# PathologyFoundation/plip

Measured on NVIDIA H100. Metric: image-text pairs/sec (224x224, 77-tok), higher is better.
Workload: dtype bf16

## Files before the change

### plip_b200/csrc/gemm_wgmma.cu

```cuda
#include "gemm.cuh"
#include "wgmma.cuh"

#include <stdio.h>
#include <stdlib.h>

namespace plip {

namespace {

constexpr int BM = 64;
constexpr int BK = 64;
constexpr int kThreads = 288;
constexpr int kConsumerWarps = 8;
constexpr uint32_t A_STAGE = BM * BK * 2;
constexpr uint32_t kStoreStageBytes = 16 * 128;

constexpr int x_boxes(int BN, int EPI) {
  return EPI != EPI_BIAS_RESID_F32 ? 2 : BN == 192 ? 3 : 2;
}

template <int BN, int EPI>
struct Cfg {
  static constexpr uint32_t B_STAGE = BN * BK * 2;
  static constexpr uint32_t STAGE = A_STAGE + B_STAGE;
  static constexpr int XBOXES = x_boxes(BN, EPI);
  static constexpr uint32_t EPI_BYTES = kConsumerWarps * XBOXES * kStoreStageBytes;
  static constexpr uint32_t BAR_BYTES = EPI == EPI_BIAS_RESID_F32 ? 512 : 256;
  static constexpr uint32_t ALIGN_SLACK = 1024;
  static constexpr int kMaxStages = (227 * 1024 - BAR_BYTES - EPI_BYTES - ALIGN_SLACK) / STAGE;
  static constexpr int STAGES = kMaxStages > 8 ? 8 : kMaxStages;
  static constexpr uint32_t SMEM_BYTES = STAGES * STAGE + EPI_BYTES + BAR_BYTES + ALIGN_SLACK;
};

struct GemmDev {
  int M, N, K;
  const float* bias;
  const float* rowscale;
  void* out;
  int ldo;
  const float* pos;
  int patches, seq;
  const float* colsum;
  const float2* stats_in;
  int n_partials;
  __nv_bfloat16* xb_out;
  float2* stats_out;
};

template <bool F16, int BN>
__device__ __forceinline__ void wgmma_ss(float (&d)[BN / 2], uint64_t adesc, uint64_t bdesc, uint32_t scale_d) {
  if constexpr (BN == 128) wgmma_ss_n128<F16>(d, adesc, bdesc, scale_d);
  else if constexpr (BN == 192) wgmma_ss_n192<F16>(d, adesc, bdesc, scale_d);
  else wgmma_ss_n256<F16>(d, adesc, bdesc, scale_d);
}

__device__ __forceinline__ float2 ln_row_terms(const GemmDev& p, int grow) {
  float s1 = 0.f, s2 = 0.f;
#pragma unroll
  for (int j = 0; j < kStatSlots; ++j) {
    const float2 t = (grow < p.M && j < p.n_partials) ? __ldg(p.stats_in + static_cast<size_t>(grow) * kStatSlots + j)
                                                      : make_float2(0.f, 0.f);
    s1 += t.x;
    s2 += t.y;
  }
  const float inv_k = 1.0f / static_cast<float>(p.K);
  const float mean = s1 * inv_k;
  const float rstd = rsqrtf(fmaxf(s2 * inv_k - mean * mean, 0.f) + kLnEps);
  return make_float2(-rstd * mean, rstd);
}

template <int BN, int EPI, bool F16>
__device__ __forceinline__ void epilogue_warp(const GemmDev& p, const CUtensorMap* tmC, float (&d)[BN / 2], uint32_t stage_smem,
                                              uint32_t& stage_sel, uint32_t xbar, int row_base, int col_base, int n_blk, int lane,
                                              float2 ln0, float2 ln1) {
  constexpr bool LN_FOLD = (EPI == EPI_LN_BIAS_BF16 || EPI == EPI_LN_BIAS_GELU_BF16);
  constexpr bool GELU = (EPI == EPI_BIAS_GELU_BF16 || EPI == EPI_LN_BIAS_GELU_BF16);
  constexpr bool HAS_BIAS = (EPI == EPI_BIAS_BF16 || EPI == EPI_BIAS_GELU_BF16 || EPI == EPI_BIAS_RESID_F32 || LN_FOLD);
  constexpr bool OUT_BF16 = (EPI == EPI_BIAS_BF16 || EPI == EPI_BIAS_GELU_BF16 || LN_FOLD);
  const int q = lane & 3, rr = lane >> 2;
  const int row0 = row_base + rr, row1 = row0 + 8;

  if constexpr (EPI == EPI_NULL) {
    float acc = 0.f;
#pragma unroll
    for (int i = 0; i < BN / 2; ++i) acc += d[i];
    if (acc == 1.2345e30f && p.M < 0) reinterpret_cast<float*>(p.out)[0] = acc;
  } else if constexpr (OUT_BF16) {
#pragma unroll
    for (int blk = 0; blk < BN / 64; ++blk) {
      const uint32_t buf = stage_smem + (stage_sel & 1u) * kStoreStageBytes;
      ++stage_sel;
      if (lane == 0) tma_store_wait_read_but_one();
      __syncwarp();
#pragma unroll
      for (int jj = 0; jj < 8; ++jj) {
        const int j = blk * 8 + jj;
        const int col = col_base + 8 * j + 2 * q;
        const float2 b = __ldg(reinterpret_cast<const float2*>(p.bias + col));
        float v00 = d[4 * j + 0], v01 = d[4 * j + 1], v10 = d[4 * j + 2], v11 = d[4 * j + 3];
        if constexpr (LN_FOLD) {
          const float2 cs = __ldg(reinterpret_cast<const float2*>(p.colsum + col));
          v00 = fmaf(ln0.y, v00, fmaf(ln0.x, cs.x, b.x));
          v01 = fmaf(ln0.y, v01, fmaf(ln0.x, cs.y, b.y));
          v10 = fmaf(ln1.y, v10, fmaf(ln1.x, cs.x, b.x));
          v11 = fmaf(ln1.y, v11, fmaf(ln1.x, cs.y, b.y));
        } else {
          v00 += b.x; v01 += b.y; v10 += b.x; v11 += b.y;
        }
        if constexpr (GELU) {
          v00 = quick_gelu(v00); v01 = quick_gelu(v01); v10 = quick_gelu(v10); v11 = quick_gelu(v11);
        }
        st_shared_b32(buf + rr * 128 + ((jj ^ rr) << 4) + q * 4, pack_op2<F16>(v00, v01));
        st_shared_b32(buf + (rr + 8) * 128 + ((jj ^ rr) << 4) + q * 4, pack_op2<F16>(v10, v11));
      }
      fence_proxy_async_smem();
      __syncwarp();
      if (lane == 0) {
        tma_store_2d(tmC, buf, col_base + blk * 64, row_base);
        tma_store_commit();
      }
    }
  } else if constexpr (EPI == EPI_BIAS_RESID_F32) {
    constexpr int kChunkCols = 32;
    constexpr int kChunks = BN / kChunkCols;
    constexpr int NB = x_boxes(BN, EPI);
    static_assert(kChunks % NB == 0, "every tile must start at staging block 0");
    constexpr int kUses = kChunks / NB;
    const bool ok0 = row0 < p.M, ok1 = row1 < p.M;
    const bool emit = p.xb_out != nullptr;
    const size_t o0 = static_cast<size_t>(ok0 ? row0 : 0) * p.ldo + col_base + 2 * q;
    const size_t o1 = o0 + 8 * static_cast<size_t>(p.ldo);
    uint32_t ph0 = 0;
    if constexpr (kUses % 2 != 0) ph0 = stage_sel++ & 1u;
    auto fetch = [&](int c) {
      if (lane == 0) {
        const uint32_t bar = xbar + 8u * (c % NB);
        mbar_arrive_expect_tx(bar, kStoreStageBytes);
        tma_load_2d(stage_smem + (c % NB) * kStoreStageBytes, tmC, bar, 2 * (col_base + c * kChunkCols), row_base);
      }
    };
    if (lane == 0) tma_store_wait_read();
    __syncwarp();
#pragma unroll
    for (int c = 0; c < NB; ++c) fetch(c);
    float st[2][2] = {};
#pragma unroll
    for (int c = 0; c < kChunks; ++c) {
      const int h = c < kChunks / 2 ? 0 : 1;
      mbar_wait(xbar + 8u * (c % NB), ph0 ^ ((c / NB) & 1u));
      const uint32_t buf = stage_smem + (c % NB) * kStoreStageBytes;
#pragma unroll
      for (int jj = 0; jj < kChunkCols / 8; ++jj) {
        const int j = c * (kChunkCols / 8) + jj;
        const int col = col_base + 8 * j + 2 * q;
        const uint32_t xoff = (((2 * jj + (q >> 1)) ^ rr) << 4) + (q & 1) * 8;
        const float2 b = __ldg(reinterpret_cast<const float2*>(p.bias + col));
        const float2 v0 = make_float2(d[4 * j + 0] + b.x, d[4 * j + 1] + b.y);
        const float2 v1 = make_float2(d[4 * j + 2] + b.x, d[4 * j + 3] + b.y);
        if (ok0) {
          const float2 x = ld_shared_f32x2(buf + rr * 128 + xoff);
          const float2 y = make_float2(x.x + v0.x, x.y + v0.y);
          st_shared_f32x2(buf + rr * 128 + xoff, y);
          if (emit) {
            *reinterpret_cast<uint32_t*>(p.xb_out + o0 + 8 * j) = pack_op2<F16>(y.x, y.y);
            st[0][0] += y.x + y.y;
            st[0][1] = fmaf(y.x, y.x, fmaf(y.y, y.y, st[0][1]));
          }
        }
        if (ok1) {
          const float2 x = ld_shared_f32x2(buf + (rr + 8) * 128 + xoff);
          const float2 y = make_float2(x.x + v1.x, x.y + v1.y);
          st_shared_f32x2(buf + (rr + 8) * 128 + xoff, y);
          if (emit) {
            *reinterpret_cast<uint32_t*>(p.xb_out + o1 + 8 * j) = pack_op2<F16>(y.x, y.y);
            st[1][0] += y.x + y.y;
            st[1][1] = fmaf(y.x, y.x, fmaf(y.y, y.y, st[1][1]));
          }
        }
      }
      fence_proxy_async_smem();
      __syncwarp();
      if (lane == 0) {
        tma_store_2d(tmC, buf, 2 * (col_base + c * kChunkCols), row_base);
        tma_store_commit();
      }
      if (c + NB < kChunks) {
        if (lane == 0) tma_store_wait_read();
        fetch(c + NB);
      }
      if (emit && (c + 1) % (kChunks / 2) == 0) {
#pragma unroll
        for (int r = 0; r < 2; ++r) {
          float a = st[r][0], b = st[r][1];
#pragma unroll
          for (int o = 1; o < 4; o <<= 1) {
            a += __shfl_xor_sync(0xffffffffu, a, o);
            b += __shfl_xor_sync(0xffffffffu, b, o);
          }
          if (q == 0 && (r == 0 ? ok0 : ok1))
            p.stats_out[static_cast<size_t>(row0 + 8 * r) * kStatSlots + 2 * n_blk + h] = make_float2(a, b);
          st[r][0] = 0.f;
          st[r][1] = 0.f;
        }
      }
    }
  } else {
    float* out = reinterpret_cast<float*>(p.out);
    const bool ok0 = row0 < p.M, ok1 = row1 < p.M;
    float rs0 = 1.f, rs1 = 1.f;
    size_t o0 = static_cast<size_t>(ok0 ? row0 : 0) * p.ldo, o1 = static_cast<size_t>(ok1 ? row1 : 0) * p.ldo;
    if constexpr (EPI == EPI_SIM_F32) {
      rs0 = ok0 ? __ldg(p.rowscale + row0) : 0.f;
      rs1 = ok1 ? __ldg(p.rowscale + row1) : 0.f;
    }
    size_t q0 = 0, q1 = 0;
    if constexpr (EPI == EPI_PATCH_F32) {
      const int r0 = ok0 ? row0 : 0, r1 = ok1 ? row1 : 0;
      const int b0 = r0 / p.patches, b1 = r1 / p.patches;
      o0 = static_cast<size_t>(b0 * p.seq + 1 + (r0 - b0 * p.patches)) * p.ldo;
      o1 = static_cast<size_t>(b1 * p.seq + 1 + (r1 - b1 * p.patches)) * p.ldo;
      q0 = static_cast<size_t>(1 + (r0 - b0 * p.patches)) * p.N;
      q1 = static_cast<size_t>(1 + (r1 - b1 * p.patches)) * p.N;
    }
#pragma unroll
    for (int j = 0; j < BN / 8; ++j) {
      const int col = col_base + 8 * j + 2 * q;
      float2 v0 = make_float2(d[4 * j + 0], d[4 * j + 1]), v1 = make_float2(d[4 * j + 2], d[4 * j + 3]);
      if constexpr (HAS_BIAS) {
        const float2 b = __ldg(reinterpret_cast<const float2*>(p.bias + col));
        v0.x += b.x; v0.y += b.y; v1.x += b.x; v1.y += b.y;
      }
      if constexpr (EPI == EPI_SIM_F32) {
        const float2 cs = __ldg(reinterpret_cast<const float2*>(p.bias + col));
        if (ok0) *reinterpret_cast<float2*>(out + o0 + col) = make_float2(v0.x * rs0 * cs.x, v0.y * rs0 * cs.y);
        if (ok1) *reinterpret_cast<float2*>(out + o1 + col) = make_float2(v1.x * rs1 * cs.x, v1.y * rs1 * cs.y);
      } else if constexpr (EPI == EPI_PATCH_F32) {
        if (ok0) {
          const float2 e = __ldg(reinterpret_cast<const float2*>(p.pos + q0 + col));
          *reinterpret_cast<float2*>(out + o0 + col) = make_float2(v0.x + e.x, v0.y + e.y);
        }
        if (ok1) {
          const float2 e = __ldg(reinterpret_cast<const float2*>(p.pos + q1 + col));
          *reinterpret_cast<float2*>(out + o1 + col) = make_float2(v1.x + e.x, v1.y + e.y);
        }
      } else {
        if (ok0) *reinterpret_cast<float2*>(out + o0 + col) = v0;
        if (ok1) *reinterpret_cast<float2*>(out + o1 + col) = v1;
      }
    }
  }
}

template <int CG, int BN, int EPI, bool F16>
__global__ void __launch_bounds__(kThreads, 1)
gemm_kernel(const __grid_constant__ CUtensorMap tmA, const __grid_constant__ CUtensorMap tmB,
            const __grid_constant__ CUtensorMap tmC, const GemmDev p) {
  using C = Cfg<BN, EPI>;
  constexpr int STAGES = C::STAGES;
  extern __shared__ uint8_t smem_raw[];
  const uint32_t smem_base = (smem_u32(smem_raw) + 1023u) & ~1023u;
  const uint32_t epi_base = smem_base + STAGES * C::STAGE;
  const uint32_t bar_base = epi_base + C::EPI_BYTES;
  auto full_bar = [&](int s) { return bar_base + 8u * s; };
  auto empty_bar = [&](int s) { return bar_base + 8u * (STAGES + s); };
  const uint32_t resid_bar = bar_base + 8u * (2 * STAGES);
  static_assert(8 * (2 * STAGES + (EPI == EPI_BIAS_RESID_F32 ? C::XBOXES * kConsumerWarps : 0)) <= C::BAR_BYTES,
                "barrier area too small");

  const int warp = threadIdx.x >> 5;
  const int lane = threadIdx.x & 31;
  const int wg = warp >> 2;
  const uint32_t cta_rank = (CG > 1) ? cluster_ctarank() : 0u;

  if (threadIdx.x == 0) {
    tma_prefetch_desc(&tmA);
    tma_prefetch_desc(&tmB);
    for (int s = 0; s < STAGES; ++s) {
      mbar_init(full_bar(s), 1);
      mbar_init(empty_bar(s), CG);
    }
    if constexpr (EPI == EPI_BIAS_RESID_F32) {
      tma_prefetch_desc(&tmC);
      for (int i = 0; i < C::XBOXES * kConsumerWarps; ++i) mbar_init(resid_bar + 8u * i, 1);
    }
    fence_mbar_init();
  }
  if constexpr (CG > 1) cluster_sync_all(); else __syncthreads();

  const int num_n_blk = p.N / BN;
  const int num_m_blk = (p.M + BM * CG - 1) / (BM * CG);
  const int num_tiles = num_m_blk * num_n_blk;
  const int num_kb = p.K / BK;
  const int tile0 = blockIdx.x / CG;
  const int tile_step = gridDim.x / CG;
  const int my_tiles = (num_tiles - tile0 + tile_step - 1) / tile_step;

  if (wg == 2) {
    if (lane == 0) {
      int s = 0;
      uint32_t ph = 0;
      for (int t = tile0; t < num_tiles; t += tile_step) {
        const int m0 = ((t / num_n_blk) * CG + cta_rank) * BM;
        const int n0 = (t % num_n_blk) * BN;
        for (int kb = 0; kb < num_kb; ++kb) {
          mbar_wait(empty_bar(s), ph ^ 1u);
          const uint32_t sa = smem_base + s * C::STAGE;
          const uint32_t sb = sa + A_STAGE;
          mbar_arrive_expect_tx(full_bar(s), C::STAGE);
          tma_load_2d(sa, &tmA, full_bar(s), kb * BK, m0);
          if constexpr (CG == 1) {
            tma_load_2d(sb, &tmB, full_bar(s), kb * BK, n0);
          } else {
            tma_load_2d_mc(sb + cta_rank * (C::B_STAGE / 2), &tmB, full_bar(s), kb * BK, n0 + cta_rank * (BN / 2), 0x3);
          }
          if (++s == STAGES) { s = 0; ph ^= 1u; }
        }
      }
    }
    __syncwarp();
  } else {
    const int wtid = threadIdx.x & 127;
    auto release = [&](int s) {
      if (wtid == 0) mbar_arrive(empty_bar(s));
      if constexpr (CG > 1) {
        if (wtid == 32) mbar_arrive_cluster(mapa_shared(empty_bar(s), cta_rank ^ 1u));
      }
    };
    float d[BN / 2];
    int s = 0;
    uint32_t ph = 0;
    auto skip_tile = [&]() {
      s += num_kb;
      ph ^= static_cast<uint32_t>(s / STAGES) & 1u;
      s %= STAGES;
    };
    uint32_t stage_sel = 0;
    const uint32_t my_turn = 1u + wg, other_turn = 2u - wg;
    const int rounds = (my_tiles + 1) / 2;
    if (wg == 1) skip_tile();
    for (int r = 0; r < rounds; ++r) {
      const int i = 2 * r + wg;
      const int t = tile0 + i * tile_step;
      const int n_blk = t % num_n_blk;
      const int m0 = ((t / num_n_blk) * CG + cta_rank) * BM;
      const int wrow = m0 + (warp & 3) * 16;
      float2 ln0 = make_float2(0.f, 1.f), ln1 = make_float2(0.f, 1.f);
      if constexpr (EPI == EPI_LN_BIAS_BF16 || EPI == EPI_LN_BIAS_GELU_BF16) {
        if (i < my_tiles) {
          ln0 = ln_row_terms(p, wrow + (lane >> 2));
          ln1 = ln_row_terms(p, wrow + (lane >> 2) + 8);
        }
      }
      if (wg == 1 || r > 0) named_barrier_sync<256>(my_turn);
      if (i >= my_tiles) break;
      int prev = -1;
      for (int kb = 0; kb < num_kb; ++kb) {
        mbar_wait(full_bar(s), ph);
        const uint32_t sa = smem_base + s * C::STAGE;
        const uint64_t adesc = make_smem_desc_sw128(sa, 1024, 16);
        const uint64_t bdesc = make_smem_desc_sw128(sa + A_STAGE, 1024, 16);
        wgmma_pin(d);
        wgmma_fence();
#pragma unroll
        for (int k = 0; k < BK / 16; ++k) wgmma_ss<F16, BN>(d, adesc + 2 * k, bdesc + 2 * k, (kb | k) != 0 ? 1u : 0u);
        wgmma_commit();
        wgmma_wait<1>();
        if (prev >= 0) release(prev);
        prev = s;
        if (++s == STAGES) { s = 0; ph ^= 1u; }
      }
      if (wg == 0 || r + 1 < rounds) named_barrier_arrive<256>(other_turn);
      wgmma_wait<0>();
      wgmma_pin(d);
      release(prev);
      skip_tile();
      epilogue_warp<BN, EPI, F16>(p, &tmC, d, epi_base + warp * C::XBOXES * kStoreStageBytes, stage_sel,
                                  resid_bar + 8u * C::XBOXES * warp, wrow,
                                  n_blk * BN, n_blk, lane, ln0, ln1);
    }
    if (lane == 0) tma_store_wait_all();
    __syncwarp();
  }
  if constexpr (CG > 1) cluster_sync_all();
}

int env_int(const char* name, int dflt) {
  const char* v = getenv(name);
  return v ? atoi(v) : dflt;
}

template <int CG, int BN, int EPI, bool F16>
int launch_inst(const GemmArgs& g, cudaStream_t stream) {
  using C = Cfg<BN, EPI>;
  auto kern = gemm_kernel<CG, BN, EPI, F16>;
  static unsigned long long configured = 0;
  static int max_groups = 0;
  if (first_use_on_device(configured)) {
    PLIP_CUDA_CHECK(cudaFuncSetAttribute(kern, cudaFuncAttributeMaxDynamicSharedMemorySize, (int)C::SMEM_BYTES));
    int dev = 0, sms = 0;
    PLIP_CUDA_CHECK(cudaGetDevice(&dev));
    PLIP_CUDA_CHECK(cudaDeviceGetAttribute(&sms, cudaDevAttrMultiProcessorCount, dev));
    max_groups = sms / CG;
    if (CG >= 2) {
      cudaLaunchConfig_t q = {};
      q.gridDim = dim3(sms / CG * CG);
      q.blockDim = dim3(kThreads);
      q.dynamicSmemBytes = C::SMEM_BYTES;
      cudaLaunchAttribute qa[1];
      qa[0].id = cudaLaunchAttributeClusterDimension;
      qa[0].val.clusterDim.x = CG; qa[0].val.clusterDim.y = 1; qa[0].val.clusterDim.z = 1;
      q.attrs = qa; q.numAttrs = 1;
      int n_clusters = 0;
      PLIP_CUDA_CHECK(cudaOccupancyMaxActiveClusters(&n_clusters, kern, &q));
      if (n_clusters > 0 && n_clusters < max_groups) max_groups = n_clusters;
    }
    PLIP_REQUIRE(max_groups > 0, "launch_gemm: no resident CTA fits (cg=%d bn=%d)", CG, BN);
  }
  CUtensorMap tmA, tmB;
  if (int rc = make_tmap_bf16_2d(&tmA, g.A, g.M, g.K, (uint64_t)g.lda * 2, BM, BK)) return rc;
  if (int rc = make_tmap_bf16_2d(&tmB, g.W, g.N, g.K, (uint64_t)g.ldw * 2, BN / CG, BK)) return rc;
  constexpr bool kOutBf16 = (EPI == EPI_BIAS_BF16 || EPI == EPI_BIAS_GELU_BF16 || EPI == EPI_LN_BIAS_BF16 ||
                             EPI == EPI_LN_BIAS_GELU_BF16);
  CUtensorMap tmC = tmA;
  if (kOutBf16)
    if (int rc = make_tmap_bf16_2d(&tmC, g.out, g.M, g.N, (uint64_t)g.ldo * 2, 16, 64)) return rc;
  if (EPI == EPI_BIAS_RESID_F32)
    if (int rc = make_tmap_bf16_2d(&tmC, g.out, g.M, 2 * (uint64_t)g.N, (uint64_t)g.ldo * 4, 16, 64)) return rc;

  GemmDev p;
  p.M = g.M; p.N = g.N; p.K = g.K;
  p.bias = g.bias; p.rowscale = g.rowscale; p.out = g.out; p.ldo = g.ldo; p.pos = g.pos;
  p.patches = g.patches; p.seq = g.seq;
  p.colsum = g.colsum; p.stats_in = g.stats_in; p.n_partials = g.n_partials;
  p.xb_out = g.xb_out; p.stats_out = g.stats_out;
  if (g.n_tiles_used) *g.n_tiles_used = 2 * (g.N / BN);

  const int num_tiles = ((g.M + BM * CG - 1) / (BM * CG)) * (g.N / BN);
  const int groups = max_groups < num_tiles ? max_groups : num_tiles;
  PLIP_CUDA_CHECK(launch_kernel(kern, dim3(groups * CG), dim3(kThreads), C::SMEM_BYTES, stream, CG, tmA, tmB, tmC, p));
  return 0;
}

template <int CG, int BN, bool F16>
int launch_epi_fmt(const GemmArgs& g, cudaStream_t stream) {
  switch (g.epi) {
    case EPI_BIAS_BF16: return launch_inst<CG, BN, EPI_BIAS_BF16, F16>(g, stream);
    case EPI_BIAS_GELU_BF16: return launch_inst<CG, BN, EPI_BIAS_GELU_BF16, F16>(g, stream);
    case EPI_BIAS_RESID_F32: return launch_inst<CG, BN, EPI_BIAS_RESID_F32, F16>(g, stream);
    case EPI_PATCH_F32: return launch_inst<CG, BN, EPI_PATCH_F32, F16>(g, stream);
    case EPI_F32: return launch_inst<CG, BN, EPI_F32, F16>(g, stream);
    case EPI_LN_BIAS_BF16: return launch_inst<CG, BN, EPI_LN_BIAS_BF16, F16>(g, stream);
    case EPI_LN_BIAS_GELU_BF16: return launch_inst<CG, BN, EPI_LN_BIAS_GELU_BF16, F16>(g, stream);
    case EPI_NULL: return launch_inst<CG, BN, EPI_NULL, F16>(g, stream);
    case EPI_SIM_F32: return launch_inst<CG, BN, EPI_SIM_F32, F16>(g, stream);
    default: set_last_error("launch_gemm: bad epilogue %d", g.epi); return -2;
  }
}
template <int CG, int BN>
int launch_epi(const GemmArgs& g, cudaStream_t stream) {
  return g.f16 ? launch_epi_fmt<CG, BN, true>(g, stream) : launch_epi_fmt<CG, BN, false>(g, stream);
}

}

int launch_gemm(const GemmArgs& g, cudaStream_t stream) {
  PLIP_REQUIRE(g.M > 0 && g.N > 0 && g.K > 0, "launch_gemm: empty problem M=%d N=%d K=%d", g.M, g.N, g.K);
  PLIP_REQUIRE(g.K % BK == 0, "launch_gemm: K=%d must be a multiple of %d", g.K, BK);
  PLIP_REQUIRE(g.N % 128 == 0 || g.N % 192 == 0, "launch_gemm: N=%d must be a multiple of 128 or 192", g.N);
  PLIP_REQUIRE((g.lda % 8) == 0 && (g.ldw % 8) == 0 && (g.ldo % 8) == 0,
               "launch_gemm: leading dimensions must be multiples of 8 elements");
  PLIP_REQUIRE((reinterpret_cast<uintptr_t>(g.A) & 15) == 0 && (reinterpret_cast<uintptr_t>(g.W) & 15) == 0 &&
               (reinterpret_cast<uintptr_t>(g.out) & 15) == 0,
               "launch_gemm: operands must be 16-byte aligned");
  if (g.epi == EPI_LN_BIAS_BF16 || g.epi == EPI_LN_BIAS_GELU_BF16)
    PLIP_REQUIRE(g.colsum && g.stats_in && g.bias && g.n_partials >= 1 && g.n_partials <= kStatSlots,
                 "launch_gemm: LayerNorm-folded epilogue needs colsum, stats and 1..%d partials", kStatSlots);
  if (g.epi == EPI_SIM_F32)
    PLIP_REQUIRE(g.bias && g.rowscale, "launch_gemm: the similarity epilogue needs row and column scales");
  if (g.epi == EPI_PATCH_F32)
    PLIP_REQUIRE(g.patches >= 1 && g.seq == g.patches + 1, "launch_gemm: patch epilogue with %d patches, %d rows",
                 g.patches, g.seq);
  if (g.xb_out || g.stats_out)
    PLIP_REQUIRE(g.epi == EPI_BIAS_RESID_F32 && g.xb_out && g.stats_out,
                 "launch_gemm: xb/stats outputs belong to the residual epilogue");
  static const int env_cg = env_int("PLIP_GEMM_CG", 0);
  static const int env_bn = env_int("PLIP_GEMM_BN", 0);
  int cg = g.force_cg ? g.force_cg : (env_cg ? env_cg : 2);
  int bn = g.force_bn ? g.force_bn : (env_bn ? env_bn : 256);
  if (g.N % bn != 0) bn = 128;
  if (!g.force_bn && g.stats_out && 2 * (g.N / bn) > kStatSlots && g.N % 256 == 0) bn = 256;
  PLIP_REQUIRE((cg == 1 || cg == 2) && (bn == 128 || bn == 256 || (bn == 192 && cg == 2)),
               "launch_gemm: bad config cg=%d bn=%d", cg, bn);
  PLIP_REQUIRE(!g.stats_out || 2 * (g.N / bn) <= kStatSlots, "launch_gemm: N=%d / BN=%d exceeds %d statistics slots",
               g.N, bn, kStatSlots);
  if (cg == 1) return bn == 256 ? launch_epi<1, 256>(g, stream) : launch_epi<1, 128>(g, stream);
  if (bn == 192) return launch_epi<2, 192>(g, stream);
  return bn == 256 ? launch_epi<2, 256>(g, stream) : launch_epi<2, 128>(g, stream);
}

}
```

Baseline: 26720.

## Prefetch residual boxes during mainloop and TMA-store bf16 residual copy for shallow-K GEMMs

For residual-add GEMMs with K up to 1024, the consumer warps issue TMA loads of the fp32 residual boxes right after the first k-block, so the loads overlap the mainloop instead of starting in the epilogue. The staging buffers are doubled. The bf16 copy of the residual stream is staged in shared memory and written with TMA stores rather than scattered 4-byte global stores, and waits are relaxed to keep one store in flight. This costs extra shared memory, which may reduce pipeline stages, and adds more complex barrier and phase bookkeeping.

```diff
diff --git a/plip_b200/csrc/gemm_wgmma.cu b/plip_b200/csrc/gemm_wgmma.cu
--- a/plip_b200/csrc/gemm_wgmma.cu
+++ b/plip_b200/csrc/gemm_wgmma.cu
@@ -15,16 +15,19 @@
 constexpr uint32_t A_STAGE = BM * BK * 2;
 constexpr uint32_t kStoreStageBytes = 16 * 128;
 
-constexpr int x_boxes(int BN, int EPI) {
-  return EPI != EPI_BIAS_RESID_F32 ? 2 : BN == 192 ? 3 : 2;
-}
-
-template <int BN, int EPI>
+constexpr int kDeepXMaxK = 1024;
+constexpr int x_boxes(int BN, int EPI, bool DEEP_X) {
+  return EPI != EPI_BIAS_RESID_F32 ? 2 : BN == 192 ? (DEEP_X ? 6 : 3) : (DEEP_X ? 4 : 2);
+}
+constexpr int xn_blocks(int EPI, bool DEEP_X) { return EPI == EPI_BIAS_RESID_F32 && DEEP_X ? 2 : 0; }
+
+template <int BN, int EPI, bool DEEP_X>
 struct Cfg {
   static constexpr uint32_t B_STAGE = BN * BK * 2;
   static constexpr uint32_t STAGE = A_STAGE + B_STAGE;
-  static constexpr int XBOXES = x_boxes(BN, EPI);
-  static constexpr uint32_t EPI_BYTES = kConsumerWarps * XBOXES * kStoreStageBytes;
+  static constexpr int XBOXES = x_boxes(BN, EPI, DEEP_X);
+  static constexpr int WARP_BLOCKS = XBOXES + xn_blocks(EPI, DEEP_X);
+  static constexpr uint32_t EPI_BYTES = kConsumerWarps * WARP_BLOCKS * kStoreStageBytes;
   static constexpr uint32_t BAR_BYTES = EPI == EPI_BIAS_RESID_F32 ? 512 : 256;
   static constexpr uint32_t ALIGN_SLACK = 1024;
   static constexpr int kMaxStages = (227 * 1024 - BAR_BYTES - EPI_BYTES - ALIGN_SLACK) / STAGE;
@@ -69,8 +72,17 @@
   return make_float2(-rstd * mean, rstd);
 }
 
-template <int BN, int EPI, bool F16>
-__device__ __forceinline__ void epilogue_warp(const GemmDev& p, const CUtensorMap* tmC, float (&d)[BN / 2], uint32_t stage_smem,
+template <int NB>
+__device__ __forceinline__ void fetch_x_box(const CUtensorMap* tmC, uint32_t stage_smem, uint32_t xbar, int c,
+                                            int col_base, int row_base) {
+  const uint32_t bar = xbar + 8u * (c % NB);
+  mbar_arrive_expect_tx(bar, kStoreStageBytes);
+  tma_load_2d(stage_smem + (c % NB) * kStoreStageBytes, tmC, bar, 2 * (col_base + c * 32), row_base);
+}
+
+template <int BN, int EPI, bool F16, bool DEEP_X>
+__device__ __forceinline__ void epilogue_warp(const GemmDev& p, const CUtensorMap* tmC, const CUtensorMap* tmXb,
+                                              float (&d)[BN / 2], uint32_t stage_smem,
                                               uint32_t& stage_sel, uint32_t xbar, int row_base, int col_base, int n_blk, int lane,
                                               float2 ln0, float2 ln1) {
   constexpr bool LN_FOLD = (EPI == EPI_LN_BIAS_BF16 || EPI == EPI_LN_BIAS_GELU_BF16);
@@ -123,37 +135,38 @@
   } else if constexpr (EPI == EPI_BIAS_RESID_F32) {
     constexpr int kChunkCols = 32;
     constexpr int kChunks = BN / kChunkCols;
-    constexpr int NB = x_boxes(BN, EPI);
+    constexpr int NB = x_boxes(BN, EPI, DEEP_X);
     static_assert(kChunks % NB == 0, "every tile must start at staging block 0");
+    static_assert(kChunks % 2 == 0, "the 16-bit copy leaves in [16 x 64] blocks of two boxes");
     constexpr int kUses = kChunks / NB;
     const bool ok0 = row0 < p.M, ok1 = row1 < p.M;
     const bool emit = p.xb_out != nullptr;
+    const uint32_t xn_smem = stage_smem + NB * kStoreStageBytes;
     const size_t o0 = static_cast<size_t>(ok0 ? row0 : 0) * p.ldo + col_base + 2 * q;
     const size_t o1 = o0 + 8 * static_cast<size_t>(p.ldo);
     uint32_t ph0 = 0;
     if constexpr (kUses % 2 != 0) ph0 = stage_sel++ & 1u;
-    auto fetch = [&](int c) {
+    if constexpr (!DEEP_X) {
       if (lane == 0) {
-        const uint32_t bar = xbar + 8u * (c % NB);
-        mbar_arrive_expect_tx(bar, kStoreStageBytes);
-        tma_load_2d(stage_smem + (c % NB) * kStoreStageBytes, tmC, bar, 2 * (col_base + c * kChunkCols), row_base);
-      }
-    };
-    if (lane == 0) tma_store_wait_read();
-    __syncwarp();
-#pragma unroll
-    for (int c = 0; c < NB; ++c) fetch(c);
+        tma_store_wait_read();
+#pragma unroll
+        for (int c = 0; c < NB; ++c) fetch_x_box<NB>(tmC, stage_smem, xbar, c, col_base, row_base);
+      }
+      __syncwarp();
+    }
     float st[2][2] = {};
 #pragma unroll
     for (int c = 0; c < kChunks; ++c) {
       const int h = c < kChunks / 2 ? 0 : 1;
       mbar_wait(xbar + 8u * (c % NB), ph0 ^ ((c / NB) & 1u));
       const uint32_t buf = stage_smem + (c % NB) * kStoreStageBytes;
+      const uint32_t xn = xn_smem + ((c / 2) % 2) * kStoreStageBytes;
 #pragma unroll
       for (int jj = 0; jj < kChunkCols / 8; ++jj) {
         const int j = c * (kChunkCols / 8) + jj;
         const int col = col_base + 8 * j + 2 * q;
         const uint32_t xoff = (((2 * jj + (q >> 1)) ^ rr) << 4) + (q & 1) * 8;
+        const uint32_t xnoff = ((((c % 2) * 4 + jj) ^ rr) << 4) + q * 4;
         const float2 b = __ldg(reinterpret_cast<const float2*>(p.bias + col));
         const float2 v0 = make_float2(d[4 * j + 0] + b.x, d[4 * j + 1] + b.y);
         const float2 v1 = make_float2(d[4 * j + 2] + b.x, d[4 * j + 3] + b.y);
@@ -162,7 +175,8 @@
           const float2 y = make_float2(x.x + v0.x, x.y + v0.y);
           st_shared_f32x2(buf + rr * 128 + xoff, y);
           if (emit) {
-            *reinterpret_cast<uint32_t*>(p.xb_out + o0 + 8 * j) = pack_op2<F16>(y.x, y.y);
+            if constexpr (DEEP_X) st_shared_b32(xn + rr * 128 + xnoff, pack_op2<F16>(y.x, y.y));
+            else *reinterpret_cast<uint32_t*>(p.xb_out + o0 + 8 * j) = pack_op2<F16>(y.x, y.y);
             st[0][0] += y.x + y.y;
             st[0][1] = fmaf(y.x, y.x, fmaf(y.y, y.y, st[0][1]));
           }
@@ -172,7 +186,8 @@
           const float2 y = make_float2(x.x + v1.x, x.y + v1.y);
           st_shared_f32x2(buf + (rr + 8) * 128 + xoff, y);
           if (emit) {
-            *reinterpret_cast<uint32_t*>(p.xb_out + o1 + 8 * j) = pack_op2<F16>(y.x, y.y);
+            if constexpr (DEEP_X) st_shared_b32(xn + (rr + 8) * 128 + xnoff, pack_op2<F16>(y.x, y.y));
+            else *reinterpret_cast<uint32_t*>(p.xb_out + o1 + 8 * j) = pack_op2<F16>(y.x, y.y);
             st[1][0] += y.x + y.y;
             st[1][1] = fmaf(y.x, y.x, fmaf(y.y, y.y, st[1][1]));
           }
@@ -182,11 +197,22 @@
       __syncwarp();
       if (lane == 0) {
         tma_store_2d(tmC, buf, 2 * (col_base + c * kChunkCols), row_base);
+        if (DEEP_X && emit && c % 2 == 1) tma_store_2d(tmXb, xn, col_base + (c / 2) * 64, row_base);
         tma_store_commit();
       }
-      if (c + NB < kChunks) {
-        if (lane == 0) tma_store_wait_read();
-        fetch(c + NB);
+      if constexpr (DEEP_X) {
+        if (c + 1 < kChunks) {
+          if (lane == 0) {
+            tma_store_wait_read_but_one();
+            if (c >= 1 && c - 1 + NB < kChunks) fetch_x_box<NB>(tmC, stage_smem, xbar, c - 1 + NB, col_base, row_base);
+          }
+          __syncwarp();
+        }
+      } else if (c + NB < kChunks) {
+        if (lane == 0) {
+          tma_store_wait_read();
+          fetch_x_box<NB>(tmC, stage_smem, xbar, c + NB, col_base, row_base);
+        }
       }
       if (emit && (c + 1) % (kChunks / 2) == 0) {
 #pragma unroll
@@ -251,11 +277,11 @@
   }
 }
 
-template <int CG, int BN, int EPI, bool F16>
+template <int CG, int BN, int EPI, bool F16, bool DEEP_X>
 __global__ void __launch_bounds__(kThreads, 1)
 gemm_kernel(const __grid_constant__ CUtensorMap tmA, const __grid_constant__ CUtensorMap tmB,
-            const __grid_constant__ CUtensorMap tmC, const GemmDev p) {
-  using C = Cfg<BN, EPI>;
+            const __grid_constant__ CUtensorMap tmC, const GemmDev p, const __grid_constant__ CUtensorMap tmXb) {
+  using C = Cfg<BN, EPI, DEEP_X>;
   constexpr int STAGES = C::STAGES;
   extern __shared__ uint8_t smem_raw[];
   const uint32_t smem_base = (smem_u32(smem_raw) + 1023u) & ~1023u;
@@ -281,6 +307,7 @@
     }
     if constexpr (EPI == EPI_BIAS_RESID_F32) {
       tma_prefetch_desc(&tmC);
+      if (DEEP_X && p.xb_out) tma_prefetch_desc(&tmXb);
       for (int i = 0; i < C::XBOXES * kConsumerWarps; ++i) mbar_init(resid_bar + 8u * i, 1);
     }
     fence_mbar_init();
@@ -364,6 +391,15 @@
 #pragma unroll
         for (int k = 0; k < BK / 16; ++k) wgmma_ss<F16, BN>(d, adesc + 2 * k, bdesc + 2 * k, (kb | k) != 0 ? 1u : 0u);
         wgmma_commit();
+        if constexpr (EPI == EPI_BIAS_RESID_F32 && DEEP_X) {
+          if (kb == 0 && lane == 0) {
+            tma_store_wait_read();
+#pragma unroll
+            for (int c = 0; c < C::XBOXES; ++c)
+              fetch_x_box<C::XBOXES>(&tmC, epi_base + warp * C::WARP_BLOCKS * kStoreStageBytes,
+                                     resid_bar + 8u * C::XBOXES * warp, c, n_blk * BN, wrow);
+          }
+        }
         wgmma_wait<1>();
         if (prev >= 0) release(prev);
         prev = s;
@@ -374,7 +410,7 @@
       wgmma_pin(d);
       release(prev);
       skip_tile();
-      epilogue_warp<BN, EPI, F16>(p, &tmC, d, epi_base + warp * C::XBOXES * kStoreStageBytes, stage_sel,
+      epilogue_warp<BN, EPI, F16, DEEP_X>(p, &tmC, &tmXb, d, epi_base + warp * C::WARP_BLOCKS * kStoreStageBytes, stage_sel,
                                   resid_bar + 8u * C::XBOXES * warp, wrow,
                                   n_blk * BN, n_blk, lane, ln0, ln1);
     }
@@ -389,10 +425,10 @@
   return v ? atoi(v) : dflt;
 }
 
-template <int CG, int BN, int EPI, bool F16>
+template <int CG, int BN, int EPI, bool F16, bool DEEP_X = false>
 int launch_inst(const GemmArgs& g, cudaStream_t stream) {
-  using C = Cfg<BN, EPI>;
-  auto kern = gemm_kernel<CG, BN, EPI, F16>;
+  using C = Cfg<BN, EPI, DEEP_X>;
+  auto kern = gemm_kernel<CG, BN, EPI, F16, DEEP_X>;
   static unsigned long long configured = 0;
   static int max_groups = 0;
   if (first_use_on_device(configured)) {
@@ -426,6 +462,9 @@
     if (int rc = make_tmap_bf16_2d(&tmC, g.out, g.M, g.N, (uint64_t)g.ldo * 2, 16, 64)) return rc;
   if (EPI == EPI_BIAS_RESID_F32)
     if (int rc = make_tmap_bf16_2d(&tmC, g.out, g.M, 2 * (uint64_t)g.N, (uint64_t)g.ldo * 4, 16, 64)) return rc;
+  CUtensorMap tmXb = tmA;
+  if (EPI == EPI_BIAS_RESID_F32 && DEEP_X && g.xb_out)
+    if (int rc = make_tmap_bf16_2d(&tmXb, g.xb_out, g.M, g.N, (uint64_t)g.ldo * 2, 16, 64)) return rc;
 
   GemmDev p;
   p.M = g.M; p.N = g.N; p.K = g.K;
@@ -437,7 +476,7 @@
 
   const int num_tiles = ((g.M + BM * CG - 1) / (BM * CG)) * (g.N / BN);
   const int groups = max_groups < num_tiles ? max_groups : num_tiles;
-  PLIP_CUDA_CHECK(launch_kernel(kern, dim3(groups * CG), dim3(kThreads), C::SMEM_BYTES, stream, CG, tmA, tmB, tmC, p));
+  PLIP_CUDA_CHECK(launch_kernel(kern, dim3(groups * CG), dim3(kThreads), C::SMEM_BYTES, stream, CG, tmA, tmB, tmC, p, tmXb));
   return 0;
 }
 
@@ -446,7 +485,9 @@
   switch (g.epi) {
     case EPI_BIAS_BF16: return launch_inst<CG, BN, EPI_BIAS_BF16, F16>(g, stream);
     case EPI_BIAS_GELU_BF16: return launch_inst<CG, BN, EPI_BIAS_GELU_BF16, F16>(g, stream);
-    case EPI_BIAS_RESID_F32: return launch_inst<CG, BN, EPI_BIAS_RESID_F32, F16>(g, stream);
+    case EPI_BIAS_RESID_F32:
+      return g.K <= kDeepXMaxK ? launch_inst<CG, BN, EPI_BIAS_RESID_F32, F16, true>(g, stream)
+                               : launch_inst<CG, BN, EPI_BIAS_RESID_F32, F16, false>(g, stream);
     case EPI_PATCH_F32: return launch_inst<CG, BN, EPI_PATCH_F32, F16>(g, stream);
     case EPI_F32: return launch_inst<CG, BN, EPI_F32, F16>(g, stream);
     case EPI_LN_BIAS_BF16: return launch_inst<CG, BN, EPI_LN_BIAS_BF16, F16>(g, stream);
@@ -481,8 +522,9 @@
     PLIP_REQUIRE(g.patches >= 1 && g.seq == g.patches + 1, "launch_gemm: patch epilogue with %d patches, %d rows",
                  g.patches, g.seq);
   if (g.xb_out || g.stats_out)
-    PLIP_REQUIRE(g.epi == EPI_BIAS_RESID_F32 && g.xb_out && g.stats_out,
-                 "launch_gemm: xb/stats outputs belong to the residual epilogue");
+    PLIP_REQUIRE(g.epi == EPI_BIAS_RESID_F32 && g.xb_out && g.stats_out &&
+                 (reinterpret_cast<uintptr_t>(g.xb_out) & 15) == 0,
+                 "launch_gemm: xb/stats outputs belong to the residual epilogue (xb 16-byte aligned)");
   static const int env_cg = env_int("PLIP_GEMM_CG", 0);
   static const int env_bn = env_int("PLIP_GEMM_BN", 0);
   int cg = g.force_cg ? g.force_cg : (env_cg ? env_cg : 2);
```

After: 27060 (median of 6 runs). +1.3%, better.
